# leimao/Voice-Converter-CycleGAN

Hardware: NVIDIA H100
Metric: CycleGAN-VC train steps/sec @ batch 256x[24,128] MCEP (higher is better)
Workload: dtype f16f8 (forward / data gradient: fp16 MMA + two e4m3 cross-term MMAs = 2 MMA units per product; weight gradient: fp16 MMA alone, 1 unit; f32 accumulate)

## Files before the change

voice-converter-cyclegan_b200/csrc/engine.cu:

```cuda
#include "../../include/cgvc.h"
#include "kernels.cuh"
#include "tc_gemm.cuh"
#include "geom.h"

#include <atomic>
#include <dlfcn.h>
#include <limits.h>
#include <stddef.h>
#include <math.h>
#include <stdarg.h>
#include <stdio.h>
#include <string.h>

#include <map>
#include <string>
#include <utility>
#include <vector>

static thread_local std::string g_create_error;

#define ADAM_B1 0.5f
#define ADAM_B2 0.999f
#define ADAM_EPS 1e-8f

// ... 371 lines not shown

static int conv_fwd(cgvc_engine* e, const Layer& L, const LayerTensors& t, const ConvIO& io, float* P, cudaStream_t st) {
  bool done = false;
  if (t.tc && io.xhi)
    RET(tc_result(e, tc_conv_fwd(*t.tc, t.precision, t.debug, io.xhi, io.xlo, io.n, io.H, io.W, L.sh, L.sw, P, st, nullptr, nullptr, packed(io)),
                  &L.a, "forward", &done));
  if (done) return 0;
  if (L.gated() && L.a.cin == 1 && io.x && !io.pk.off && L.a.cout % 4 == 0 && 256 % (L.a.cout / 2) == 0) {
    GatherGeom g = fwd_geom(io.n, io.H, io.W, L.a.kh, L.a.kw, L.sh, L.sw);
    CK(launch_conv_c1_fwd(g, io.x, t.ka, t.kg, t.ba, t.bg, L.a.cout, P, st));
    return 0;
  }
  RET(conv_fwd_simt(e, t.ka, t.ba, L.a, L.sh, L.sw, io, P, L.width(), 0, st));
  if (L.gated()) RET(conv_fwd_simt(e, t.kg, t.bg, L.g, L.sh, L.sw, io, P, L.width(), L.a.cout, st));
  return 0;
}

static int conv_dgrad(cgvc_engine* e, const Layer& L, const LayerTensors& t, const ConvIO& io, const float* dP, PlanePair dp, float* dx,
                      int accumulate, cudaStream_t st, const TcBwdFuse* fuse = nullptr, bool* fused = nullptr) {
  bool done = false;
  if (t.tc && dp.hi)
    RET(tc_result(e, tc_conv_dgrad(*t.tc, t.precision, t.debug, dp.hi, dp.lo, io.n, io.H, io.W, L.sh, L.sw, dx, accumulate, st, fuse, fused,
                                   packed(io)), &L.a, "data gradient", &done));
  if (done) return 0;
  RET(conv_dgrad_simt(e, t.ka, L.a, L.sh, L.sw, io.n, io.H, io.W, dP, L.width(), 0, dx, accumulate, st, packed(io)));
  if (L.gated()) RET(conv_dgrad_simt(e, t.kg, L.g, L.sh, L.sw, io.n, io.H, io.W, dP, L.width(), L.a.cout, dx, 1, st, packed(io)));
  return 0;
}

static int conv_wgrad(cgvc_engine* e, const Layer& L, const LayerTensors& t, const ConvIO& io, const float* dP, PlanePair dp, cudaStream_t st,
                      const DetSlab* det) {
  bool done = false;
  if (t.tc && dp.hi && io.xhi)
    RET(tc_result(e, tc_conv_wgrad(*t.tc, t.precision, t.wgrad16, io.xhi, io.xlo, dp.hi, dp.lo, io.n, io.H, io.W, L.sh, L.sw, t.dka, t.dkg,
                                   st, det, packed(io)), &L.a, "weight gradient", &done));
  if (done) return 0;
  RET(conv_wgrad_simt(e, t.dka, L.a, L.sh, L.sw, io, dP, L.width(), 0, st, det));
  if (L.gated()) RET(conv_wgrad_simt(e, t.dkg, L.g, L.sh, L.sw, io, dP, L.width(), L.a.cout, st, det));
  return 0;
}

static PostParams post_params(const cgvc_engine* e, const Layer& L, const LayerTensors& t, const ConvIO& io, const GLAct& A,
                              int rows_per_sample_out, bool keep_y, float* scratch, const float* resid = nullptr) {
  PostParams q; memset(&q, 0, sizeof q);
  q.scratch = scratch;
  q.p = A.P; q.ldp = L.width(); q.Cc = L.a.cout; q.B = io.n; q.sh = L.shuffle;
  q.R = rows_per_sample_out * L.shuffle; q.C = L.a.cout / L.shuffle;
  q.has_in = L.has_in; q.has_gate = L.gated();
  q.beta_a = t.beta_a; q.gamma_a = t.gamma_a; q.beta_g = t.beta_g; q.gamma_g = t.gamma_g;
  q.resid = resid;
  q.y = (keep_y || !A.Yhi) ? A.Y : nullptr;
  q.stats = L.has_in ? A.stats : nullptr; q.y_hi = A.Yhi; q.y_lo = A.Ylo;
  q.qmode = t.precision == CGVC_PREC_F16F8;
  q.sat = sat_act(e);
  if (io.pk.off && L.has_in && io.seg_out) {
    const long long frames = (long long)io.pk.div * io.W, view_rows = q.R;
    q.B = io.pk.n; q.R = (int)(view_rows * io.pk.max_len / frames);
    q.seg = PackGeom{io.seg_out, io.pk.n, 1, q.R}; q.seg_rows = view_rows;
  } else if (io.pk.off && L.has_in) {
    const long long view_rows = q.R;
    const int div = (int)((long long)io.pk.div * io.W / view_rows);
    q.seg = PackGeom{io.pk.off, io.pk.n, div, io.pk.max_len}; q.seg_rows = view_rows;
    q.B = io.pk.n; q.R = io.pk.max_len / div;
  }
  return q;
}

// ... 236 lines not shown
                    float* dx, int accumulate, cudaStream_t st, const Layer* up, const LayerTensors* ut, const GLAct* upA) {
  const int other = 1 - w.cur;
  TcBwdFuse f;
  const bool fuse = up && w.fuse && dp.hi;
  if (fuse) f = bwd_fuse(*up, *ut, *upA, in.W, w.pb[other]);
  bool fused = false;
  RET(conv_dgrad(e, L, t, in, dP, dp, dx, accumulate, st, fuse ? &f : nullptr, &fused));
  if (fused) w.have = other;
  return 0;
}

static int layer_backward(cgvc_engine* e, BwdWalk& w, const Layer& L, const GLAct& A, const ConvIO& in, const float* dy,
                          int rows_per_sample_out, bool wgrad, float* dx, int accumulate, cudaStream_t st,
                          const Layer* up = nullptr, const GLAct* upA = nullptr) {
  const LayerTensors t = layer_tensors(e, L, wgrad);
  PostBwdParams q;
  RET(layer_dp(e, w, L, t, A, dy, in.n, rows_per_sample_out, st, q, &in));
  const PlanePair dp{q.dp_hi, q.dp_lo};
  if (wgrad) RET(run_wgrad(w.S, dp.hi != nullptr, st, [&](cudaStream_t ws) { return conv_wgrad(e, L, t, in, q.dp, dp, ws, det_of(w.S)); }));
  if (!dx) return 0;
  LayerTensors ut{};
  if (up) ut = layer_tensors(e, *up, wgrad);
  return layer_dx(e, w, L, t, in, q.dp, dp, dx, accumulate, st, up, &ut, upA);
}

static int o1_edge_backward(cgvc_engine* e, const GenNet& N, const float* d_out, const __nv_bfloat16* uhi, const __nv_bfloat16* ulo, int n,
                            int T, PlanePair dz, float* du, const BwdScratch& S, cudaStream_t st, const long long* off = nullptr, int n_off = 0) {
  const int nf = e->cfg.num_features;
  float* Gm = e->G();
  const TcLayer& O = e->tcw.layers[N.o1f_slot];
  CK(launch_im2col_taps(d_out, (long long)n * T, T, nf, N.o1.a.kw, -1, edge_cpad(N.o1.a.kw * nf), e->cfg.precision == CGVC_PREC_F16F8,
                        dz.hi, dz.lo, st, off, n_off, sat_grad(e), ufl_grad(e)));
  RET(run_wgrad(S, true, st, [&](cudaStream_t ws) {
    return tc_result(e, tc_conv_wgrad(O, e->cfg.precision, e->tcw.wgrad16, uhi, ulo, dz.hi, dz.lo, n, 1, T, 1, 1, Gm + N.o1.a.k, nullptr, ws,
                                      det_of(S)),
                     &N.o1.a, "weight gradient (tap-lowered)"); }));
  RET(tc_result(e, tc_conv_dgrad(O, e->cfg.precision, e->tcw.debug, dz.hi, dz.lo, n, 1, T, 1, 1, du, 0, st), &N.o1.a,
                "data gradient (tap-lowered)"));
  return 0;
}

static int h1_edge_backward(cgvc_engine* e, const GenNet& N, const __nv_bfloat16* xchi, const __nv_bfloat16* xclo, PlanePair dp, int n,
                            int T, float* dz, float* dx, const BwdScratch& S, cudaStream_t st, const long long* off = nullptr, int n_off = 0) {
  const int nf = e->cfg.num_features;
  float* Gm = e->G();
  const TcLayer& H = e->tcw.layers[N.h1c_slot];
  RET(run_wgrad(S, true, st, [&](cudaStream_t ws) {
    return tc_result(e, tc_conv_wgrad(H, e->cfg.precision, e->tcw.wgrad16, xchi, xclo, dp.hi, dp.lo, n, 1, T, 1, 1, Gm + N.h1.a.k,
                                      Gm + N.h1.g.k, ws, det_of(S)),
                     &N.h1.a, "weight gradient (tap-lowered)"); }));
  if (dz) RET(tc_result(e, tc_conv_dgrad(H, e->cfg.precision, e->tcw.debug, dp.hi, dp.lo, n, 1, T, 1, 1, dz, 0, st), &N.h1.a,
                        "data gradient (tap-lowered)"));
  if (dz && dx) CK(launch_col2im_taps(dz, N.h1.a.kw * nf, (long long)n * T, T, nf, N.h1.a.kw, -1, nullptr, dx, st, off, n_off));
  return 0;
}

static int generator_backward(cgvc_engine* e, const GenNet& N, const GenActs& A, const float* d_out_cl, float* d_in_cl,
                              const BwdScratch& S, cudaStream_t st) {
  const bool packed = A.off != nullptr;
  const int n = packed ? 1 : A.n, T = packed ? (int)A.rows : A.T, nf = e->cfg.num_features;
  float* Gm = e->G();
  auto at = [&](const float* x, const __nv_bfloat16* hi, const __nv_bfloat16* lo, int W) {
    ConvIO io; io.x = x; io.xhi = hi; io.xlo = lo; io.n = n; io.H = 1; io.W = W;
    if (packed) io.pk = PackGeom{A.off, A.n, (int)(A.rows / W), A.max_len};
    return io;
  };
  auto of = [&](const GLAct& a, int W) { return at(a.Y, a.Yhi, a.Ylo, W); };
  BwdWalk w(S, e->opt.fuse_bwd && !packed && !e->opt.deterministic && !sat_grad(e) && !side_on(S) && tc_enabled(e) && S.dPhi && S.dP2hi &&
               A.r[0].h1.Yhi && A.r[0].h2.Yhi);
  const bool edge = edge_on(e, N) && A.xchi && A.z;
  CK(launch_colsum(d_out_cl, (long long)n * T, nf, 0, nf, Gm + N.o1.a.b, st, det_of(S)));
  const ConvIO u2 = of(A.u[1], T);
  if (edge && u2.xhi && S.dPhi) {
    RET(o1_edge_backward(e, N, d_out_cl, u2.xhi, u2.xlo, n, T, dp_planes(w, st), S.bufA, S, st, A.off, A.n));
  } else {
    const LayerTensors t = layer_tensors(e, N.o1, true);
    PlanePair dp{nullptr, nullptr};
    if (t.tc && u2.xhi && S.dPhi) {
      dp = dp_planes(w, st);
      CK(tc_split_planes(e->cfg.precision, d_out_cl, (long long)n * T, nf, dp.hi, dp.lo, st, sat_grad(e), ufl_grad(e)));
    }
// ... 1788 lines not shown
```

voice-converter-cyclegan_b200/csrc/tc_gemm.cu:

```cuda
#include "tc_gemm.cuh"
#include "geom.h"
#include "kernels.cuh"
#include "wgmma.cuh"

#include <cuda.h>
#include <stdint.h>
#include <stdio.h>
#include <string.h>

namespace {

typedef CUresult (*EncodeTiledFn)(CUtensorMap*, CUtensorMapDataType, cuuint32_t, void*, const cuuint64_t*, const cuuint64_t*,
                                  const cuuint32_t*, const cuuint32_t*, CUtensorMapInterleave, CUtensorMapSwizzle,
                                  CUtensorMapL2promotion, CUtensorMapFloatOOBfill);
EncodeTiledFn get_encoder() {
  static EncodeTiledFn fn = nullptr;
  if (!fn) {
    void* p = nullptr; cudaDriverEntryPointQueryResult q;
    if (cudaGetDriverEntryPoint("cuTensorMapEncodeTiled", &p, cudaEnableDefault, &q) == cudaSuccess && q == cudaDriverEntryPointSuccess)
      fn = (EncodeTiledFn)p;
  }
  return fn;
}
bool make_tmap3(CUtensorMap* m, const void* base, uint64_t d0, uint64_t d1, uint64_t d2, uint32_t b1) {
// ... 141 lines not shown
__device__ __forceinline__ RowPos nt_row(const TcNTParams& p, long long m) {
  RowPos r;
  r.y = (int)fdiv((uint32_t)m, p.div_bw);
  const uint32_t rem = (uint32_t)m - (uint32_t)r.y * p.div_bw.d;
  r.b = (int)fdiv(rem, p.div_w);
  r.x = (int)(rem - (uint32_t)r.b * p.div_w.d);
  return r;
}
template <int PK = 0>
__device__ __forceinline__ uint32_t nt_tile_taps(const TcNTParams& p, long long m0, long long M) {
  const long long m1 = m0 + 127 < M ? m0 + 127 : M - 1;
  if constexpr (PK == 2) {
    const int dout = p.pk.div * p.g.sx;
    const Pack2Pos a = pack2_pos(p.pk, p.g.Hy, dout, m0), b = pack2_pos(p.pk, p.g.Hy, dout, m1);
    return a.u == b.u ? gather_tap_mask(p.g, a.y, b.y) : (1u << p.g.ntaps) - 1u;
  }
  return gather_tap_mask(p.g, nt_row(p, m0).y, nt_row(p, m1).y);
}

struct TcTNParams {
  GatherGeom g;
  const __nv_bfloat16 *x_hi, *x_lo; int x_ld; int C;
  const __nv_bfloat16 *g_hi, *g_lo; int g_ld; int N;
  float* dw_a; float* dw_g; int n_split;
  int ksplit;
  FastDiv div_hw, div_w;
  CUtensorMap tm_g_hi, tm_g_lo;
  const uint8_t *x8_hi, *x8_lo;
  const uint8_t *g8_hi, *g8_lo;
  int w16;
  int fold_n;
  float* part; long long part_k, numel_a;
  PackGeom pk;
};

__device__ __forceinline__ float* tn_dst(float* base, int slab, int C, int c, int ncols, int col, int fold_n) {
  if (fold_n) { const int t = col / fold_n; return base + ((long long)t * C + c) * fold_n + (col - t * fold_n); }
  return base + ((long long)slab * C + c) * ncols + col;
}

constexpr int kProducerThreads = 128;


template <int BN, int NPL>
struct NTCfg {
  static constexpr int A_PLANE = 128 * 128;
  static constexpr int B_PLANE = BN * 128;
  static constexpr int PLANES = NPL == 2 ? 2 : 1;
  static constexpr int STAGE = PLANES * (A_PLANE + B_PLANE);
  static constexpr int STAGES = (192 * 1024) / STAGE;
  static constexpr int SMEM = STAGES * STAGE + 1024;
  static_assert(STAGES * STAGE >= 128 * BN * 4, "the finished fp32 tile is staged over the pipeline stages");
};

template <int BN>
__device__ __forceinline__ int acc_off(int r, int n) { return r * BN + (n & ~31) + ((((n >> 2) & 7) ^ (r & 7)) << 2) + (n & 3); }
template <int BN>
__device__ __forceinline__ void acc_ld32(const float* acc, int r, int col, uint32_t (&v)[32]) {
#pragma unroll
  for (int c = 0; c < 8; ++c) {
    const float4 x = *reinterpret_cast<const float4*>(acc + r * BN + col + ((c ^ (r & 7)) << 2));
    v[4 * c] = __float_as_uint(x.x); v[4 * c + 1] = __float_as_uint(x.y); v[4 * c + 2] = __float_as_uint(x.z); v[4 * c + 3] = __float_as_uint(x.w);
  }
}

__device__ __forceinline__ float warp_colsum32(float (&t)[32], int lane) {
#pragma unroll
// ... 753 lines not shown
      const int r0 = wg * 64 + (tw >> 5) * 16 + ((tw & 31) >> 2), c0 = 2 * (tw & 3);
      if constexpr (EPI == 0) {
        if (!(p.debug & 3)) nt_store_fragments<BN, PK>(p, d, M, m0, n0, r0, c0);
      } else {
        consumer_bar();
        if (!(p.debug & 2)) {
#pragma unroll
          for (int j = 0; j < BN / 8; ++j) {
            *reinterpret_cast<float2*>(acc_s + acc_off<BN>(r0, 8 * j + c0)) = make_float2(d[4 * j], d[4 * j + 1]);
            *reinterpret_cast<float2*>(acc_s + acc_off<BN>(r0 + 8, 8 * j + c0)) = make_float2(d[4 * j + 2], d[4 * j + 3]);
          }
        }
        consumer_bar();
        nt_tile_epilogue<BN, NPL, EPI>(p, M, m0, n0, cw & 3, lane, epi_stage[cw], epi_rowp[cw], epi_bc[cw], epi_xch[wg], acc_s, wg, 2);
        fence_proxy_async();
        __syncwarp();
        if (lane == 0) mbar_arrive(&acc_free_bar);
      }
    }
  }
}

#define CGVC_Q_WGRAD_SHIFT 12
template <int NPL, int W16>
struct TNCfg {
  static constexpr int A_PLANE = 64 * 256;
  static constexpr int B_PLANE = 64 * 512;
  static constexpr int PLANES = (NPL == 1 || W16) ? 1 : 2;
  static constexpr int STAGE = PLANES * (A_PLANE + B_PLANE);
  static constexpr int STAGES = (192 * 1024) / STAGE;
  static constexpr int SMEM = STAGES * STAGE + 1024;
};

template <int NPL, int W16, int DET, int PK = 0>
__global__ void __launch_bounds__(kNTThreads, 1)
tc_gg_tn_kernel(const __grid_constant__ TcTNParams p) {
  static_assert(W16 == 0 || NPL == 3, "the fp16-only weight gradient is a form of CGVC_PREC_F16F8");
  using Cfg = TNCfg<NPL, W16>;
  constexpr int S = Cfg::STAGES;
  constexpr int BN = 256;
  extern __shared__ uint8_t smem_raw[];
  __shared__ __align__(8) uint64_t full_bar[S], empty_bar[S];

  const uint32_t smem_base = (smem_u32(smem_raw) + 1023u) & ~1023u;
  const int warp = threadIdx.x >> 5, lane = threadIdx.x & 31;
  const GatherGeom& g = p.g;
  const long long M = (long long)g.B * g.Hy * g.Wx;
  const int HW = g.Hy * g.Wx;
  const int n_tiles = (p.g_ld + BN - 1) / BN, c_tiles = (p.x_ld + 127) / 128;
  const int num_items = n_tiles * c_tiles * g.ntaps * p.ksplit;
  constexpr int pass0 = (NPL == 3 && !W16) ? 0 : 1;
  long long chunk_rows = (M + p.ksplit - 1) / p.ksplit;
  chunk_rows = (chunk_rows + 63) / 64 * 64;

  struct Item { int n0, c0, tap, ks; long long mbeg, mend; int num_kb; };
  auto decode = [&](int item) -> Item {
    Item w;
    int n_t = item % n_tiles; int t1 = item / n_tiles;
    int c_t = t1 % c_tiles; int t2 = t1 / c_tiles;
    w.tap = t2 % g.ntaps; const int ks = t2 / g.ntaps; w.ks = ks;
    w.n0 = n_t * BN; w.c0 = c_t * 128;
    w.mbeg = (long long)ks * chunk_rows;
    w.mend = (w.mbeg + chunk_rows < M) ? w.mbeg + chunk_rows : M;
    w.num_kb = w.mend > w.mbeg ? (int)((w.mend - w.mbeg + 63) / 64) : 0;
    return w;
  };

  if (threadIdx.x == 0) {
    for (int s = 0; s < S; ++s) { mbar_init(&full_bar[s], kProducerThreads + 1); mbar_init(&empty_bar[s], 8); }
    fence_barrier_init();
    tma_prefetch_desc(&p.tm_g_hi);
    if (NPL == 2) tma_prefetch_desc(&p.tm_g_lo);
  }
  __syncthreads();

  if (warp < 4) {
    const int t = threadIdx.x;
    const int chunk = t & 7, rsub = t >> 3;
    int stage = 0; uint32_t phase = 0;
    for (int item = blockIdx.x; item < num_items; item += gridDim.x) {
      const Item w = decode(item);
      for (int pass = pass0; pass < 2; ++pass)
      for (int kb = 0; kb < w.num_kb; ++kb) {
        mbar_wait(&empty_bar[stage], phase ^ 1);
        const uint32_t sA = smem_base + stage * Cfg::STAGE;
        const uint32_t sB = sA + Cfg::PLANES * Cfg::A_PLANE;
        long long xoff[4];
#pragma unroll
        for (int i = 0; i < 4; ++i) {
          const long long m = w.mbeg + (long long)kb * 64 + rsub + 16 * i;
          xoff[i] = -1;
          if (m < w.mend) {
            if constexpr (PK == 2) {
              const Pack2Pos o = pack2_pos(p.pk, g.Hy, p.pk.div * g.sx, m);
              const long long r = pack2_row(o.o0, o.o1, g.Hs, p.pk.div, o.y * g.sy + g.oy[w.tap], o.x * g.sx + g.ox[w.tap]);
              if (r >= 0) xoff[i] = r * p.x_ld + w.c0 + chunk * 8;
            } else if constexpr (PK) {
              const int dout = p.pk.div * g.sx;
              const int u = pack_find(p.pk.off, p.pk.n, m * dout);
              const long long o0 = __ldg(p.pk.off + u), o1 = __ldg(p.pk.off + u + 1);
              const int xx = (int)(m - o0 / dout) * g.sx + g.ox[w.tap];
              if (xx >= 0 && xx < (int)((o1 - o0) / p.pk.div)) xoff[i] = (o0 / p.pk.div + xx) * p.x_ld + w.c0 + chunk * 8;
            } else {
              const uint32_t mu = (uint32_t)m;
              int b = (int)fdiv(mu, p.div_hw); int rem = (int)(mu - (uint32_t)b * (uint32_t)HW);
              int y = (int)fdiv((uint32_t)rem, p.div_w); int x = rem - y * g.Wx;
              int yy = y * g.sy + g.oy[w.tap], xx = x * g.sx + g.ox[w.tap];
              if (yy >= 0 && yy < g.Hs && xx >= 0 && xx < g.Ws)
                xoff[i] = ((long long)(b * g.Hs + yy) * g.Ws + xx) * p.x_ld + w.c0 + chunk * 8;
            }
          }
        }
        if (NPL == 3 && pass == 0) {
#pragma unroll
          for (int i = 0; i < 4; ++i) {
            const int kr = rsub + 16 * i;
            const uint32_t so = sw128(kr, chunk);
#pragma unroll
            for (int a = 0; a < 2; ++a) {
              const bool ok = xoff[i] >= 0 && (w.c0 + a * 64) < p.x_ld;
              uint2 vh = make_uint2(0u, 0u), vl = make_uint2(0u, 0u);
              if (ok) { vh = __ldg(reinterpret_cast<const uint2*>(p.x8_hi + xoff[i] + a * 64)); vl = __ldg(reinterpret_cast<const uint2*>(p.x8_lo + xoff[i] + a * 64)); }
              st_shared16(sA + a * 8192 + so, e4m3x8_to_f16x8(vh));
              st_shared16(sA + Cfg::A_PLANE + a * 8192 + so, e4m3x8_to_f16x8(vl));
            }
            const long long m = w.mbeg + (long long)kb * 64 + kr;
#pragma unroll
            for (int a = 0; a < 4; ++a) {
              const int col = w.n0 + a * 64 + chunk * 8;
              const bool ok = m < w.mend && col < p.g_ld;
              uint2 vh = make_uint2(0u, 0u), vl = make_uint2(0u, 0u);
              if (ok) { vh = __ldg(reinterpret_cast<const uint2*>(p.g8_hi + m * p.g_ld + col)); vl = __ldg(reinterpret_cast<const uint2*>(p.g8_lo + m * p.g_ld + col)); }
              st_shared16(sB + a * 8192 + so, e4m3x8_to_f16x8(vh));
              st_shared16(sB + Cfg::B_PLANE + a * 8192 + so, e4m3x8_to_f16x8(vl));
            }
          }
          fence_proxy_async();
          if (t == 0) mbar_expect_tx(&full_bar[stage], 0);
          mbar_arrive(&full_bar[stage]);
        } else {
          if (t == 0) {
            const int row0 = (int)(w.mbeg + (long long)kb * 64);
            int natoms = 0;
#pragma unroll
            for (int a = 0; a < 4; ++a) natoms += (w.n0 + a * 64) < p.g_ld ? 1 : 0;
            mbar_expect_tx(&full_bar[stage], (NPL == 2 ? 2 : 1) * natoms * 8192);
#pragma unroll
            for (int a = 0; a < 4; ++a) {
              if ((w.n0 + a * 64) < p.g_ld) {
                tma_load3(sB + a * 8192, &p.tm_g_hi, w.n0 + a * 64, row0, 0, &full_bar[stage]);
                if (NPL == 2) tma_load3(sB + Cfg::B_PLANE + a * 8192, &p.tm_g_lo, w.n0 + a * 64, row0, 0, &full_bar[stage]);
              }
            }
          }
#pragma unroll
          for (int i = 0; i < 4; ++i) {
            const uint32_t so = sw128(rsub + 16 * i, chunk);
#pragma unroll
            for (int a = 0; a < 2; ++a) {
              const bool ok = xoff[i] >= 0 && (w.c0 + a * 64) < p.x_ld;
              const long long off = ok ? xoff[i] + a * 64 : 0;
              cp_async16(sA + a * 8192 + so, p.x_hi + off, ok ? 16u : 0u);
              if (NPL == 2) cp_async16(sA + Cfg::A_PLANE + a * 8192 + so, p.x_lo + off, ok ? 16u : 0u);
            }
          }
          cp_async_arrive_noinc(&full_bar[stage]);
        }
        if (++stage == S) { stage = 0; phase ^= 1; }
      }
    }
  } else {
    const int cw = warp - 4;
    const int wg = cw >> 2;
    const int tw = threadIdx.x - 128 * (wg + 1);
    int stage = 0; uint32_t phase = 0;
    for (int item = blockIdx.x; item < num_items; item += gridDim.x) {
      const Item w = decode(item);
      if (w.num_kb == 0) continue;
      float d[BN / 2];
#pragma unroll
      for (int i = 0; i < BN / 2; ++i) d[i] = 0.f;
      int prev = -1;
      if constexpr (NPL == 3 && !W16) {
        consume_stages<BN, MMA_F16_CROSS, 1, Cfg>(d, w.num_kb, stage, phase, prev, full_bar, empty_bar, smem_base, wg, lane);
        rescale_acc(d, 1.f / (float)(1 << CGVC_Q_WGRAD_SHIFT));
        consume_stages<BN, MMA_F16, 1, Cfg>(d, w.num_kb, stage, phase, prev, full_bar, empty_bar, smem_base, wg, lane);
      } else if constexpr (NPL == 3) {
// ... 251 lines not shown
  }
  else if (p.pk.off) {
    if (epi != 0 || p.g.B != 1 || p.g.Hy != 1) return cudaErrorInvalidValue;
    const int npl = precision == 3 ? 3 : x3 ? 2 : 1;
    if (bn == 256)      { if (npl == 3) LAUNCH_NT(256, 3, 0, 1); else if (npl == 2) LAUNCH_NT(256, 2, 0, 1); else LAUNCH_NT(256, 1, 0, 1); }
    else if (bn == 128) { if (npl == 3) LAUNCH_NT(128, 3, 0, 1); else if (npl == 2) LAUNCH_NT(128, 2, 0, 1); else LAUNCH_NT(128, 1, 0, 1); }
    else                { if (npl == 3) LAUNCH_NT(32, 3, 0, 1);  else if (npl == 2) LAUNCH_NT(32, 2, 0, 1);  else LAUNCH_NT(32, 1, 0, 1); }
  }
  else {
    const bool ta = nt_tma_maps(p, precision == 3 ? 3 : x3 ? 2 : 1);
#define LAUNCH_NT_D(BN_, NPL_, EPI_) do { if (ta) LAUNCH_NT(BN_, NPL_, EPI_, 0, 1); else LAUNCH_NT(BN_, NPL_, EPI_); } while (0)
    if (precision == 3) {
      if (epi == 1)       LAUNCH_NT_D(256, 3, 1);
      else if (epi == 2)  LAUNCH_NT_D(256, 3, 2);
      else if (epi == 5)  LAUNCH_NT_D(256, 3, 5);
      else if (epi != 0)  return cudaErrorInvalidValue;
      else if (bn == 256) LAUNCH_NT_D(256, 3, 0);
      else if (bn == 128) LAUNCH_NT_D(128, 3, 0);
      else                LAUNCH_NT_D(32, 3, 0);
    }
    else if (epi == 1)  { if (x3) LAUNCH_NT_D(256, 2, 1); else LAUNCH_NT_D(256, 1, 1); }
    else if (epi == 2)  { if (x3) LAUNCH_NT_D(256, 2, 2); else LAUNCH_NT_D(256, 1, 2); }
    else if (epi == 3)  { if (x3) LAUNCH_NT_D(256, 2, 3); else LAUNCH_NT_D(256, 1, 3); }
    else if (epi == 4)  { if (x3) LAUNCH_NT_D(256, 2, 4); else LAUNCH_NT_D(256, 1, 4); }
    else if (epi == 5)  { if (x3) LAUNCH_NT_D(256, 2, 5); else LAUNCH_NT_D(256, 1, 5); }
    else if (bn == 256) { if (x3) LAUNCH_NT_D(256, 2, 0); else LAUNCH_NT_D(256, 1, 0); }
    else if (bn == 128) { if (x3) LAUNCH_NT_D(128, 2, 0); else LAUNCH_NT_D(128, 1, 0); }
    else                { if (x3) LAUNCH_NT_D(32, 2, 0);  else LAUNCH_NT_D(32, 1, 0); }
#undef LAUNCH_NT_D
  }
#undef LAUNCH_NT
  prof_end(st);
  return cudaGetLastError();
}

cudaError_t launch_tn(TcTNParams p, int precision, cudaStream_t st, const DetSlab* det) {
  const long long M = (long long)p.g.B * p.g.Hy * p.g.Wx;
  if (M == 0) return cudaSuccess;
  if (M >= (1ll << 31)) return cudaErrorInvalidValue;
  const int tiles = ((p.g_ld + 255) / 256) * ((p.x_ld + 127) / 128) * p.g.ntaps;
  const int nsm = num_sms();
  long long maxsplit = M / 1024; if (maxsplit < 1) maxsplit = 1; if (maxsplit > 32) maxsplit = 32;
  int ksplit = 1; double best = 0.0;
  for (int ks = 1; ks <= (int)maxsplit; ++ks) {
    long long items = (long long)tiles * ks;
    double eff = (double)items / (double)(((items + nsm - 1) / nsm) * nsm);
    if (items < nsm) eff *= 0.5;
    if (eff > best + 0.02) { best = eff; ksplit = ks; }
  }
  const long long numel = (long long)p.g.ntaps * p.C * p.N;
  auto chunk_of = [&](int ks) { return ((M + ks - 1) / ks + 63) / 64 * 64; };
  if (det && det->p)
    while (ksplit > 1 && ((long long)ksplit * numel > det->cap || (long long)(ksplit - 1) * chunk_of(ksplit) >= M)) --ksplit;
  const bool det_split = det && det->p && ksplit > 1;
  if (det_split) { p.part = det->p; p.part_k = numel; p.numel_a = (long long)p.g.ntaps * p.C * p.n_split; }
  p.ksplit = ksplit;
  p.div_hw = make_fastdiv((uint32_t)(p.g.Hy * p.g.Wx)); p.div_w = make_fastdiv((uint32_t)p.g.Wx);
  const long long items = (long long)tiles * ksplit;
  dim3 grid((unsigned)(items < nsm ? items : nsm));
  cudaError_t e;
  ++g_cgvc_launches;
  prof_begin(st, 2.0 * (double)M * p.N * p.g.ntaps * p.C, 1, M, p.N, p.g.ntaps * p.C);
#define LAUNCH_TN(NPL_, W16_, DET_, ...)                                                                      \
  do {                                                                                                        \
    e = set_smem(tc_gg_tn_kernel<NPL_, W16_, DET_, ##__VA_ARGS__>, TNCfg<NPL_, W16_>::SMEM);                  \
    if (e != cudaSuccess) return e;                                                                           \
    tc_gg_tn_kernel<NPL_, W16_, DET_, ##__VA_ARGS__><<<grid, kNTThreads, TNCfg<NPL_, W16_>::SMEM, st>>>(p);   \
  } while (0)
  if (p.pk.off && (p.g.Hy > 1 || p.g.Hs > 1)) {
    if (p.g.B != 1) return cudaErrorInvalidValue;
    if (det_split) {
      if (precision == 3) { if (p.w16) LAUNCH_TN(3, 1, 1, 2); else LAUNCH_TN(3, 0, 1, 2); }
      else if (precision == 1) LAUNCH_TN(2, 0, 1, 2);
      else                     LAUNCH_TN(1, 0, 1, 2);
    } else {
      if (precision == 3) { if (p.w16) LAUNCH_TN(3, 1, 0, 2); else LAUNCH_TN(3, 0, 0, 2); }
      else if (precision == 1) LAUNCH_TN(2, 0, 0, 2);
      else                     LAUNCH_TN(1, 0, 0, 2);
    }
  } else if (p.pk.off) {
    if (p.g.B != 1 || p.g.Hy != 1) return cudaErrorInvalidValue;
    if (det_split) {
      if (precision == 3) { if (p.w16) LAUNCH_TN(3, 1, 1, 1); else LAUNCH_TN(3, 0, 1, 1); }
      else if (precision == 1) LAUNCH_TN(2, 0, 1, 1);
      else                     LAUNCH_TN(1, 0, 1, 1);
    } else {
      if (precision == 3) { if (p.w16) LAUNCH_TN(3, 1, 0, 1); else LAUNCH_TN(3, 0, 0, 1); }
      else if (precision == 1) LAUNCH_TN(2, 0, 0, 1);
      else                     LAUNCH_TN(1, 0, 0, 1);
    }
  } else if (det_split) {
    if (precision == 3) { if (p.w16) LAUNCH_TN(3, 1, 1); else LAUNCH_TN(3, 0, 1); }
    else if (precision == 1) LAUNCH_TN(2, 0, 1);
    else                     LAUNCH_TN(1, 0, 1);
  } else {
    if (precision == 3) { if (p.w16) LAUNCH_TN(3, 1, 0); else LAUNCH_TN(3, 0, 0); }
    else if (precision == 1) LAUNCH_TN(2, 0, 0);
    else                     LAUNCH_TN(1, 0, 0);
  }
#undef LAUNCH_TN
  prof_end(st);
  if (!det_split) return cudaGetLastError();
  e = cudaGetLastError();
  if (e != cudaSuccess) return e;
  return launch_reduce_parts(p.part, ksplit, numel, DetSegs{{p.dw_a, p.dw_g}, {0, p.numel_a}, {p.numel_a, p.dw_g ? numel - p.numel_a : 0}}, st);
}

inline int ru(int v, int m) { return (v + m - 1) / m * m; }
inline int Ntot(const TcLayer& L) { return L.cout * (L.gated ? 2 : 1); }
inline int cin_k(const TcLayer& L) { return ru(L.cin, 64); }
inline int cin_n(const TcLayer& L) { return ru(L.cin, 128); }
inline int nt_k(const TcLayer& L) { return ru(Ntot(L), 64); }
inline int nt_n(const TcLayer& L) { return ru(Ntot(L), 128); }
inline int cin_q(const TcLayer& L) { return ru(L.cin, 128); }
inline int nt_q(const TcLayer& L) { return ru(Ntot(L), 128); }
inline size_t wq_elems(const TcLayer& L) { return (size_t)L.kh * L.kw * nt_n(L) * cin_q(L); }
inline size_t wdq_elems(const TcLayer& L) { return (size_t)L.kh * L.kw * cin_n(L) * nt_q(L); }
inline size_t wf_elems(const TcLayer& L) { return (size_t)L.kh * L.kw * nt_n(L) * cin_k(L); }
inline size_t wd_elems(const TcLayer& L) { return (size_t)L.kh * L.kw * cin_n(L) * nt_k(L); }
inline int layer_perm(const TcLayer& L) {
  if (L.gated && L.shuffle == 2 && L.cout % 128 == 0) return 2;
  return (L.gated && L.cout % 128 == 0) ? 1 : 0;
}
inline bool layer_ok(const TcLayer& L) {
  if (L.fold && (L.gated || L.kh * L.kw != 1 || L.cout % L.fold || (L.cout / L.fold) % 4)) return false;
  return L.kh * L.kw <= CGVC_MAX_TAPS && Ntot(L) % 4 == 0;
}
inline bool layer_ok_q(const TcLayer& L) { return layer_ok(L) && L.cin % 4 == 0; }


bool make_layer_maps(TcLayer& L) {
// ... 93 lines not shown
  int epi = 0;
  if (fuse && fuse->R > 0 && gs.size() == 1 && H == 1 && sh == 1 && sw == 1 && (fuse->R == 32 || fuse->R == 64 || fuse->R == 128) &&
      gs[0].Wx == fuse->R && cin_n(L) % 256 == 0 && L.cin == cin_n(L) && fuse->bp && fuse->stats && fuse->dp_hi && fuse->dp_lo && fuse->gamma_a &&
      (fuse->gated ? (fuse->gamma_g && fuse->beta_a && fuse->beta_g) : (dx != nullptr)) && precision != 3)
    epi = fuse->gated ? 3 : 4;
  for (const GatherGeom& g : gs) {
    TcNTParams p; memset(&p, 0, sizeof p);
    p.g = g;
    if (pk) {
      p.pk = *pk; p.pk.div = pk->div * sw;
    }
    p.a_hi = dPhi; p.a_lo = dPlo; p.a_ld = nt_k(L); p.C = nt_k(L);
    p.b_hi = L.wd_hi; p.b_lo = L.wd_lo; p.Nw = cin_n(L); p.N = L.cin;
    p.dst = dx; p.d_ld = L.cin; p.bias = nullptr; p.accumulate = accumulate;
    p.tm_b_hi = L.tm_d_hi; p.tm_b_lo = L.tm_d_lo; p.debug = debug;
    if (precision == 3) {
      p.a_ld = nt_q(L); p.C = nt_q(L); p.a_lo = nullptr;
      p.a8_hi = reinterpret_cast<const uint8_t*>(dPlo); p.a8_lo = p.a8_hi + (size_t)g.B * g.Hs * g.Ws * nt_q(L);
      p.tm_b_hi = L.tm_dq16; p.tm_b8_hi = L.tm_dq8hi; p.tm_b8_lo = L.tm_dq8lo;
    }
    if (epi) {
      p.R = fuse->R; p.C_out = L.cin; p.stats = const_cast<float*>(fuse->stats);
      p.gamma_a = fuse->gamma_a; p.beta_a = fuse->beta_a; p.gamma_g = fuse->gamma_g; p.beta_g = fuse->beta_g;
      p.bp = fuse->bp; p.bp_ld = fuse->bp_ld; p.dp_hi = fuse->dp_hi; p.dp_lo = fuse->dp_lo; p.dp_ld = fuse->dp_ld;
      p.dbeta_a = fuse->dbeta_a; p.dgamma_a = fuse->dgamma_a; p.dbeta_g = fuse->dbeta_g; p.dgamma_g = fuse->dgamma_g;
    }
    cudaError_t e = launch_nt(p, precision, st, epi);
    if (e != cudaSuccess) return (int)e;
  }
  if (fused_out) *fused_out = epi != 0;
  return 0;
}

int tc_conv_wgrad(const TcLayer& L, int precision, int w16, const __nv_bfloat16* xhi, const __nv_bfloat16* xlo,
                  const __nv_bfloat16* dPhi, const __nv_bfloat16* dPlo, int n, int H, int W, int sh, int sw,
                  float* dwa, float* dwg, cudaStream_t st, const DetSlab* det, const PackGeom* pk) {
  if (!layer_ok(L) || (precision == 3 && !layer_ok_q(L))) return TC_UNSUPPORTED;
  if (pk && (n != 1 || (H == 1 && L.kh != 1))) return (int)cudaErrorInvalidValue;
  TcTNParams p; memset(&p, 0, sizeof p);
  if (pk) p.pk = *pk;
  p.w16 = (precision == 3 && w16) ? 1 : 0;
  p.fold_n = L.fold ? L.cout / L.fold : 0;
  p.g = fwd_geom(n, H, W, L.kh, L.kw, sh, sw);
  p.x_hi = xhi; p.x_lo = xlo; p.x_ld = cin_k(L); p.C = L.cin;
  p.g_hi = dPhi; p.g_lo = dPlo; p.g_ld = nt_k(L); p.N = Ntot(L);
  p.dw_a = dwa; p.dw_g = dwg; p.n_split = L.cout;
  const long long M = (long long)p.g.B * p.g.Hy * p.g.Wx;
  if (precision == 3) {
    const long long rows_in = (long long)n * H * W;
    p.x_ld = cin_q(L); p.g_ld = nt_q(L); p.x_lo = p.g_lo = nullptr;
    p.x8_hi = reinterpret_cast<const uint8_t*>(xlo); p.x8_lo = p.x8_hi + rows_in * p.x_ld;
    p.g8_hi = reinterpret_cast<const uint8_t*>(dPlo); p.g8_lo = p.g8_hi + M * p.g_ld;
    if (!make_tmap3_t(&p.tm_g_hi, dPhi, CU_TENSOR_MAP_DATA_TYPE_FLOAT16, 2, (uint64_t)p.g_ld, (uint64_t)M, 1, 64, 64))
      return (int)cudaErrorInvalidValue;
  } else if (!make_tmap3(&p.tm_g_hi, dPhi, (uint64_t)nt_k(L), (uint64_t)M, 1, 64) || !make_tmap3(&p.tm_g_lo, dPlo, (uint64_t)nt_k(L), (uint64_t)M, 1, 64)) {
    return (int)cudaErrorInvalidValue;
  }
  return (int)launch_tn(p, precision, st, det);
}

int tc_register(TcWeights& w, size_t ka, size_t kg, size_t ba, size_t bg, int kh, int kw, int cin, int cout, int gated, int shuffle, int fold) {
  TcLayer L{}; L.ka = ka; L.kg = kg; L.ba = ba; L.bg = bg; L.kh = kh; L.kw = kw; L.cin = cin; L.cout = cout; L.gated = gated; L.shuffle = shuffle; L.fold = fold;
  w.layers.push_back(L);
  return (int)w.layers.size() - 1;
}

static cudaError_t tc_init_kernels();

int tc_alloc(TcWeights& w, int precision, bool train) {
  { cudaError_t ie = tc_init_kernels(); if (ie != cudaSuccess) return (int)ie; }
  w.quant = precision == 3;
  w.quant_bwd = w.quant && train;
  w.wgrad16 = w.quant;
  size_t total = 0;
// ... 51 lines not shown
      err = cudaMalloc(&w.prep_jobs, jobs.size() * sizeof(PrepJob));
      if (err != cudaSuccess) return (int)err;
      err = cudaMemcpy(w.prep_jobs, jobs.data(), jobs.size() * sizeof(PrepJob), cudaMemcpyHostToDevice);
      if (err != cudaSuccess) return (int)err;
    }
  }
  w.ready = false;
  return 0;
}

static cudaError_t tc_init_kernels() {
  cudaError_t e;
#define INIT_NT(BN_, NPL_, EPI_) if ((e = set_smem(tc_gg_nt_kernel<BN_, NPL_, EPI_>, NTCfg<BN_, NPL_>::SMEM)) != cudaSuccess) return e;
  INIT_NT(256, 2, 0) INIT_NT(256, 1, 0) INIT_NT(128, 2, 0) INIT_NT(128, 1, 0) INIT_NT(32, 2, 0) INIT_NT(32, 1, 0)
  INIT_NT(256, 2, 1) INIT_NT(256, 1, 1) INIT_NT(256, 2, 2) INIT_NT(256, 1, 2)
  INIT_NT(256, 2, 3) INIT_NT(256, 1, 3) INIT_NT(256, 2, 4) INIT_NT(256, 1, 4) INIT_NT(256, 2, 5) INIT_NT(256, 1, 5)
  INIT_NT(256, 3, 0) INIT_NT(128, 3, 0) INIT_NT(32, 3, 0) INIT_NT(256, 3, 1) INIT_NT(256, 3, 2) INIT_NT(256, 3, 5)
#undef INIT_NT
#define INIT_NT(BN_, NPL_, EPI_) if ((e = set_smem(tc_gg_nt_kernel<BN_, NPL_, EPI_, 0, 1>, NTCfg<BN_, NPL_>::SMEM)) != cudaSuccess) return e;
  INIT_NT(256, 2, 0) INIT_NT(256, 1, 0) INIT_NT(128, 2, 0) INIT_NT(128, 1, 0) INIT_NT(32, 2, 0) INIT_NT(32, 1, 0)
  INIT_NT(256, 2, 1) INIT_NT(256, 1, 1) INIT_NT(256, 2, 2) INIT_NT(256, 1, 2)
  INIT_NT(256, 2, 3) INIT_NT(256, 1, 3) INIT_NT(256, 2, 4) INIT_NT(256, 1, 4) INIT_NT(256, 2, 5) INIT_NT(256, 1, 5)
  INIT_NT(256, 3, 0) INIT_NT(128, 3, 0) INIT_NT(32, 3, 0) INIT_NT(256, 3, 1) INIT_NT(256, 3, 2) INIT_NT(256, 3, 5)
#undef INIT_NT
#define INIT_NT_PK(BN_, NPL_, PK_) if ((e = set_smem(tc_gg_nt_kernel<BN_, NPL_, 0, PK_>, NTCfg<BN_, NPL_>::SMEM)) != cudaSuccess) return e;
  INIT_NT_PK(256, 1, 1) INIT_NT_PK(256, 2, 1) INIT_NT_PK(256, 3, 1) INIT_NT_PK(128, 1, 1) INIT_NT_PK(128, 2, 1) INIT_NT_PK(128, 3, 1)
  INIT_NT_PK(32, 1, 1) INIT_NT_PK(32, 2, 1) INIT_NT_PK(32, 3, 1)
  INIT_NT_PK(256, 1, 2) INIT_NT_PK(256, 2, 2) INIT_NT_PK(256, 3, 2) INIT_NT_PK(128, 1, 2) INIT_NT_PK(128, 2, 2) INIT_NT_PK(128, 3, 2)
  INIT_NT_PK(32, 1, 2) INIT_NT_PK(32, 2, 2) INIT_NT_PK(32, 3, 2)
#undef INIT_NT_PK
#define INIT_TN(NPL_, W16_, DET_) if ((e = set_smem(tc_gg_tn_kernel<NPL_, W16_, DET_>, TNCfg<NPL_, W16_>::SMEM)) != cudaSuccess) return e;
  INIT_TN(3, 1, 0) INIT_TN(3, 0, 0) INIT_TN(2, 0, 0) INIT_TN(1, 0, 0)
  INIT_TN(3, 1, 1) INIT_TN(3, 0, 1) INIT_TN(2, 0, 1) INIT_TN(1, 0, 1)
#define INIT_TN_PK(NPL_, W16_, DET_, PK_) if ((e = set_smem(tc_gg_tn_kernel<NPL_, W16_, DET_, PK_>, TNCfg<NPL_, W16_>::SMEM)) != cudaSuccess) return e;
  INIT_TN_PK(3, 1, 0, 1) INIT_TN_PK(3, 0, 0, 1) INIT_TN_PK(2, 0, 0, 1) INIT_TN_PK(1, 0, 0, 1)
  INIT_TN_PK(3, 1, 1, 1) INIT_TN_PK(3, 0, 1, 1) INIT_TN_PK(2, 0, 1, 1) INIT_TN_PK(1, 0, 1, 1)
  INIT_TN_PK(3, 1, 0, 2) INIT_TN_PK(3, 0, 0, 2) INIT_TN_PK(2, 0, 0, 2) INIT_TN_PK(1, 0, 0, 2)
  INIT_TN_PK(3, 1, 1, 2) INIT_TN_PK(3, 0, 1, 2) INIT_TN_PK(2, 0, 1, 2) INIT_TN_PK(1, 0, 1, 2)
#undef INIT_TN_PK
#undef INIT_TN
  return cudaSuccess;
}

void tc_free(TcWeights& w) {
  if (w.pool) cudaFree(w.pool);
  if (w.prep_jobs) cudaFree(w.prep_jobs);
  w.pool = nullptr; w.prep_jobs = nullptr; w.ready = false;
}

static int refresh_jobs(TcWeights& w, const float* params, int j0, int j1, cudaStream_t st) {
  if (j1 <= j0) return 0;
  const int b0 = w.job_first[j0], nb = w.job_first[j1] - b0;
  ++g_cgvc_launches;
  prep_weights_q_all_kernel<<<(unsigned)nb, 256, 0, st>>>(params, (const PrepJob*)w.prep_jobs, j0, j1, b0);
  return (int)cudaGetLastError();
}

int tc_refresh_weights(TcWeights& w, const float* params, cudaStream_t st) {
  if (!w.pool) return 0;
  const bool batched = w.prep_batched && w.prep_jobs;
  for (TcLayer& L : w.layers) {
    if (batched && L.wq16) continue;
    int r = tc_refresh_layer(L, params + L.ka, params + L.kg, params + L.ba, params + L.bg, st);
    if (r != 0) return r;
  }
  if (batched) { int r = refresh_jobs(w, params, 0, (int)w.job_ka.size(), st); if (r != 0) return r; }
// ... 87 lines not shown
```

voice-converter-cyclegan_b200/csrc/tc_gemm.cuh:

```cuda
#pragma once
#include <cuda.h>
#include <cuda_runtime.h>
#include <cuda_bf16.h>
#include <stddef.h>
#include <vector>
#include "kernels.cuh"

#define TC_UNSUPPORTED (-12345)

struct TcLayer {
  size_t ka, kg, ba, bg;
  int kh, kw, cin, cout, gated;
  int shuffle;
  int fold;
  __nv_bfloat16 *wf_hi, *wf_lo;
  __nv_bfloat16 *wd_hi, *wd_lo;
  float* bias;
  CUtensorMap tm_f_hi, tm_f_lo;
  CUtensorMap tm_d_hi, tm_d_lo;
  void* wq16; uint8_t *wq8hi, *wq8lo;
  CUtensorMap tm_q16, tm_q8hi, tm_q8lo;
  void* wdq16; uint8_t *wdq8hi, *wdq8lo;
  CUtensorMap tm_dq16, tm_dq8hi, tm_dq8lo;
};
// ... 18 lines not shown
  const float *gamma_a, *beta_a, *gamma_g, *beta_g;
  float* stats;
  const float* resid;
  float* y; __nv_bfloat16 *y_hi, *y_lo;
};

struct TcBwdFuse {
  int R;
  int gated;
  const float* bp; int bp_ld;
  const float* stats;
  const float *gamma_a, *beta_a, *gamma_g, *beta_g;
  __nv_bfloat16 *dp_hi, *dp_lo; int dp_ld;
  float *dbeta_a, *dgamma_a, *dbeta_g, *dgamma_g;
};

int tc_register(TcWeights& w, size_t ka, size_t kg, size_t ba, size_t bg, int kh, int kw, int cin, int cout, int gated, int shuffle = 1, int fold = 0);
int tc_alloc(TcWeights& w, int precision, bool train);
void tc_free(TcWeights& w);
int tc_refresh_weights(TcWeights& w, const float* params, cudaStream_t st);
int tc_refresh_layer(TcLayer& L, const float* ka, const float* kg, const float* ba, const float* bg, cudaStream_t st);
int tc_refresh_weights_range(TcWeights& w, const float* params, size_t begin, size_t end, cudaStream_t st);
void tc_layer_dims(const TcWeights& w, int slot, int dims[7]);
int tc_layer_plane(const TcWeights& w, int slot, const char* name, const void** p, size_t* bytes);

cudaError_t tc_split_planes(int precision, const float* x, long long rows, int C, __nv_bfloat16* hi, __nv_bfloat16* lo, cudaStream_t st,
                            unsigned long long* sat = nullptr, unsigned long long* ufl = nullptr);

int tc_conv_fwd(const TcLayer& L, int precision, int debug, const __nv_bfloat16* xhi, const __nv_bfloat16* xlo, int n, int H, int W,
                int sh, int sw, float* P, cudaStream_t st, const TcFuse* fuse = nullptr, bool* fused = nullptr, const PackGeom* pk = nullptr);
int tc_conv_dgrad(const TcLayer& L, int precision, int debug, const __nv_bfloat16* dPhi, const __nv_bfloat16* dPlo, int n, int H, int W,
                  int sh, int sw, float* dx, int accumulate, cudaStream_t st, const TcBwdFuse* fuse = nullptr, bool* fused = nullptr,
                  const PackGeom* pk = nullptr);
int tc_conv_wgrad(const TcLayer& L, int precision, int w16, const __nv_bfloat16* xhi, const __nv_bfloat16* xlo,
                  const __nv_bfloat16* dPhi, const __nv_bfloat16* dPlo, int n, int H, int W, int sh, int sw,
                  float* dwa, float* dwg, cudaStream_t st, const DetSlab* det = nullptr,
                  const PackGeom* pk = nullptr);

void tc_profile_enable(int on);
bool tc_profile_is_on();
int tc_profile_collect(double ms[3], double flops[3], long long launches[3]);
int tc_profile_launches(double* ms, double* flops, long long* meta4, int capacity, int* n_out);
```

Measured before the change: 10.74.

## Load weight-gradient activation tiles with TMA instead of producer-thread gathers

Adds a TMA variant of the weight-gradient TN kernel in which one producer warp issues 4D tensor-map loads for the activation planes and 3D loads for the gradient planes, replacing the four-warp manual gather and swizzled shared-memory stores. It is used for dense (unpacked) layers when the geometry fits the box constraints and the precision does not need e4m3 widening, including the fp16-only weight-gradient mode. This is meant to cut producer instruction and register overhead and let the async copy engine keep the pipeline fed. It also threads a debug flag through so activation loads can be skipped for timing experiments, and it adds more kernel instantiations plus tensor-map setup on the host for each launch.

```diff
diff --git a/voice-converter-cyclegan_b200/csrc/engine.cu b/voice-converter-cyclegan_b200/csrc/engine.cu
--- a/voice-converter-cyclegan_b200/csrc/engine.cu
+++ b/voice-converter-cyclegan_b200/csrc/engine.cu
@@ -427,7 +427,7 @@
                       const DetSlab* det) {
   bool done = false;
   if (t.tc && dp.hi && io.xhi)
-    RET(tc_result(e, tc_conv_wgrad(*t.tc, t.precision, t.wgrad16, io.xhi, io.xlo, dp.hi, dp.lo, io.n, io.H, io.W, L.sh, L.sw, t.dka, t.dkg,
+    RET(tc_result(e, tc_conv_wgrad(*t.tc, t.precision, t.debug, t.wgrad16, io.xhi, io.xlo, dp.hi, dp.lo, io.n, io.H, io.W, L.sh, L.sw, t.dka, t.dkg,
                                    st, det, packed(io)), &L.a, "weight gradient", &done));
   if (done) return 0;
   RET(conv_wgrad_simt(e, t.dka, L.a, L.sh, L.sw, io, dP, L.width(), 0, st, det));
@@ -730,7 +730,7 @@
   CK(launch_im2col_taps(d_out, (long long)n * T, T, nf, N.o1.a.kw, -1, edge_cpad(N.o1.a.kw * nf), e->cfg.precision == CGVC_PREC_F16F8,
                         dz.hi, dz.lo, st, off, n_off, sat_grad(e), ufl_grad(e)));
   RET(run_wgrad(S, true, st, [&](cudaStream_t ws) {
-    return tc_result(e, tc_conv_wgrad(O, e->cfg.precision, e->tcw.wgrad16, uhi, ulo, dz.hi, dz.lo, n, 1, T, 1, 1, Gm + N.o1.a.k, nullptr, ws,
+    return tc_result(e, tc_conv_wgrad(O, e->cfg.precision, e->tcw.debug, e->tcw.wgrad16, uhi, ulo, dz.hi, dz.lo, n, 1, T, 1, 1, Gm + N.o1.a.k, nullptr, ws,
                                       det_of(S)),
                      &N.o1.a, "weight gradient (tap-lowered)"); }));
   RET(tc_result(e, tc_conv_dgrad(O, e->cfg.precision, e->tcw.debug, dz.hi, dz.lo, n, 1, T, 1, 1, du, 0, st), &N.o1.a,
@@ -744,7 +744,7 @@
   float* Gm = e->G();
   const TcLayer& H = e->tcw.layers[N.h1c_slot];
   RET(run_wgrad(S, true, st, [&](cudaStream_t ws) {
-    return tc_result(e, tc_conv_wgrad(H, e->cfg.precision, e->tcw.wgrad16, xchi, xclo, dp.hi, dp.lo, n, 1, T, 1, 1, Gm + N.h1.a.k,
+    return tc_result(e, tc_conv_wgrad(H, e->cfg.precision, e->tcw.debug, e->tcw.wgrad16, xchi, xclo, dp.hi, dp.lo, n, 1, T, 1, 1, Gm + N.h1.a.k,
                                       Gm + N.h1.g.k, ws, det_of(S)),
                      &N.h1.a, "weight gradient (tap-lowered)"); }));
   if (dz) RET(tc_result(e, tc_conv_dgrad(H, e->cfg.precision, e->tcw.debug, dp.hi, dp.lo, n, 1, T, 1, 1, dz, 0, st), &N.h1.a,
diff --git a/voice-converter-cyclegan_b200/csrc/tc_gemm.cu b/voice-converter-cyclegan_b200/csrc/tc_gemm.cu
--- a/voice-converter-cyclegan_b200/csrc/tc_gemm.cu
+++ b/voice-converter-cyclegan_b200/csrc/tc_gemm.cu
@@ -197,7 +197,10 @@
   int fold_n;
   float* part; long long part_k, numel_a;
   PackGeom pk;
+  int debug;
+  CUtensorMap tm_x_hi, tm_x_lo;
 };
+static_assert(sizeof(TcTNParams) <= 4096, "kernel parameters are limited to 4 KB");
 
 __device__ __forceinline__ float* tn_dst(float* base, int slab, int C, int c, int ncols, int col, int fold_n) {
   if (fold_n) { const int t = col / fold_n; return base + ((long long)t * C + c) * fold_n + (col - t * fold_n); }
@@ -1017,10 +1020,11 @@
   static constexpr int SMEM = STAGES * STAGE + 1024;
 };
 
-template <int NPL, int W16, int DET, int PK = 0>
+template <int NPL, int W16, int DET, int PK = 0, int TA = 0>
 __global__ void __launch_bounds__(kNTThreads, 1)
 tc_gg_tn_kernel(const __grid_constant__ TcTNParams p) {
   static_assert(W16 == 0 || NPL == 3, "the fp16-only weight gradient is a form of CGVC_PREC_F16F8");
+  static_assert(!TA || (!PK && (NPL != 3 || W16)), "the TMA form is dense and loads the planes as they are (no e4m3 widening)");
   using Cfg = TNCfg<NPL, W16>;
   constexpr int S = Cfg::STAGES;
   constexpr int BN = 256;
@@ -1052,14 +1056,54 @@
   };
 
   if (threadIdx.x == 0) {
-    for (int s = 0; s < S; ++s) { mbar_init(&full_bar[s], kProducerThreads + 1); mbar_init(&empty_bar[s], 8); }
+    for (int s = 0; s < S; ++s) { mbar_init(&full_bar[s], TA ? 1 : kProducerThreads + 1); mbar_init(&empty_bar[s], 8); }
     fence_barrier_init();
     tma_prefetch_desc(&p.tm_g_hi);
     if (NPL == 2) tma_prefetch_desc(&p.tm_g_lo);
+    if (TA) { tma_prefetch_desc(&p.tm_x_hi); if (NPL == 2) tma_prefetch_desc(&p.tm_x_lo); }
   }
   __syncthreads();
 
-  if (warp < 4) {
+  if (TA && warp < 4) {
+    if (warp == 0) {
+      const int box_rows = (g.Hy == 1 || g.Wx >= 64) ? 64 : g.Wx;
+      const int nbox = 64 / box_rows;
+      const uint32_t x_bytes = (p.debug & 4) ? 0u : (uint32_t)Cfg::PLANES * Cfg::A_PLANE;
+      int stage = 0; uint32_t phase = 0;
+      for (int item = blockIdx.x; item < num_items; item += gridDim.x) {
+        const Item w = decode(item);
+        for (int kb = 0; kb < w.num_kb; ++kb) {
+          mbar_wait(&empty_bar[stage], phase ^ 1);
+          const uint32_t sA = smem_base + stage * Cfg::STAGE;
+          const uint32_t sB = sA + Cfg::PLANES * Cfg::A_PLANE;
+          const int row0 = (int)(w.mbeg + (long long)kb * 64);
+          if (lane == 0) {
+            int natoms = 0;
+#pragma unroll
+            for (int a = 0; a < 4; ++a) natoms += (w.n0 + a * 64) < p.g_ld ? 1 : 0;
+            mbar_expect_tx(&full_bar[stage], Cfg::PLANES * natoms * 8192 + x_bytes);
+          }
+          __syncwarp();
+          if (lane < 4) {
+            if ((w.n0 + lane * 64) < p.g_ld) {
+              tma_load3(sB + lane * 8192, &p.tm_g_hi, w.n0 + lane * 64, row0, 0, &full_bar[stage]);
+              if (NPL == 2) tma_load3(sB + Cfg::B_PLANE + lane * 8192, &p.tm_g_lo, w.n0 + lane * 64, row0, 0, &full_bar[stage]);
+            }
+          } else if (x_bytes && lane < 4 + 2 * nbox) {
+            const int j = (lane - 4) >> 1, a = (lane - 4) & 1;
+            const uint32_t mu = (uint32_t)(row0 + j * box_rows);
+            const int b = (int)fdiv(mu, p.div_hw); const int rem = (int)(mu - (uint32_t)b * (uint32_t)HW);
+            const int y = (int)fdiv((uint32_t)rem, p.div_w); const int x = rem - y * g.Wx;
+            const int c0 = w.c0 + a * 64, xs = x * g.sx + g.ox[w.tap], ys = y * g.sy + g.oy[w.tap];
+            const uint32_t dst = sA + a * 8192 + j * box_rows * 128;
+            tma_load4(dst, &p.tm_x_hi, c0, xs, ys, b, &full_bar[stage]);
+            if (NPL == 2) tma_load4(dst + Cfg::A_PLANE, &p.tm_x_lo, c0, xs, ys, b, &full_bar[stage]);
+          }
+          if (++stage == S) { stage = 0; phase ^= 1; }
+        }
+      }
+    }
+  } else if (warp < 4) {
     const int t = threadIdx.x;
     const int chunk = t & 7, rsub = t >> 3;
     int stage = 0; uint32_t phase = 0;
@@ -1103,6 +1147,7 @@
             const uint32_t so = sw128(kr, chunk);
 #pragma unroll
             for (int a = 0; a < 2; ++a) {
+              if (p.debug & 4) break;
               const bool ok = xoff[i] >= 0 && (w.c0 + a * 64) < p.x_ld;
               uint2 vh = make_uint2(0u, 0u), vl = make_uint2(0u, 0u);
               if (ok) { vh = __ldg(reinterpret_cast<const uint2*>(p.x8_hi + xoff[i] + a * 64)); vl = __ldg(reinterpret_cast<const uint2*>(p.x8_lo + xoff[i] + a * 64)); }
@@ -1138,6 +1183,7 @@
               }
             }
           }
+          if (!(p.debug & 4))
 #pragma unroll
           for (int i = 0; i < 4; ++i) {
             const uint32_t so = sw128(rsub + 16 * i, chunk);
@@ -1455,6 +1501,14 @@
 #undef LAUNCH_NT
   prof_end(st);
   return cudaGetLastError();
+}
+
+static bool tn_tma_maps(TcTNParams& p, int npl) {
+  const GatherGeom& g = p.g;
+  const int wx = g.Wx < 64 ? g.Wx : 64;
+  if (g.Wx < 8 || 64 % wx || g.Wx % wx || wx * g.sx > 256 || g.sx > 8) return false;
+  const uint32_t bx = (uint32_t)(wx * g.sx), nb = g.Hy == 1 ? (uint32_t)(64 / wx) : 1u;
+  return make_tmap_act(&p.tm_x_hi, p.x_hi, 2, p.x_ld, g, bx, nb) && (npl != 2 || make_tmap_act(&p.tm_x_lo, p.x_lo, 2, p.x_ld, g, bx, nb));
 }
 
 cudaError_t launch_tn(TcTNParams p, int precision, cudaStream_t st, const DetSlab* det) {
@@ -1512,14 +1566,19 @@
       else if (precision == 1) LAUNCH_TN(2, 0, 0, 1);
       else                     LAUNCH_TN(1, 0, 0, 1);
     }
-  } else if (det_split) {
-    if (precision == 3) { if (p.w16) LAUNCH_TN(3, 1, 1); else LAUNCH_TN(3, 0, 1); }
-    else if (precision == 1) LAUNCH_TN(2, 0, 1);
-    else                     LAUNCH_TN(1, 0, 1);
   } else {
-    if (precision == 3) { if (p.w16) LAUNCH_TN(3, 1, 0); else LAUNCH_TN(3, 0, 0); }
-    else if (precision == 1) LAUNCH_TN(2, 0, 0);
-    else                     LAUNCH_TN(1, 0, 0);
+    const bool ta = (precision != 3 || p.w16) && tn_tma_maps(p, precision == 1 ? 2 : 1);
+#define LAUNCH_TN_D(NPL_, W16_, DET_) do { if (ta) LAUNCH_TN(NPL_, W16_, DET_, 0, 1); else LAUNCH_TN(NPL_, W16_, DET_); } while (0)
+    if (det_split) {
+      if (precision == 3) { if (p.w16) LAUNCH_TN_D(3, 1, 1); else LAUNCH_TN(3, 0, 1); }
+      else if (precision == 1) LAUNCH_TN_D(2, 0, 1);
+      else                     LAUNCH_TN_D(1, 0, 1);
+    } else {
+      if (precision == 3) { if (p.w16) LAUNCH_TN_D(3, 1, 0); else LAUNCH_TN(3, 0, 0); }
+      else if (precision == 1) LAUNCH_TN_D(2, 0, 0);
+      else                     LAUNCH_TN_D(1, 0, 0);
+    }
+#undef LAUNCH_TN_D
   }
 #undef LAUNCH_TN
   prof_end(st);
@@ -1679,14 +1738,14 @@
   return 0;
 }
 
-int tc_conv_wgrad(const TcLayer& L, int precision, int w16, const __nv_bfloat16* xhi, const __nv_bfloat16* xlo,
+int tc_conv_wgrad(const TcLayer& L, int precision, int debug, int w16, const __nv_bfloat16* xhi, const __nv_bfloat16* xlo,
                   const __nv_bfloat16* dPhi, const __nv_bfloat16* dPlo, int n, int H, int W, int sh, int sw,
                   float* dwa, float* dwg, cudaStream_t st, const DetSlab* det, const PackGeom* pk) {
   if (!layer_ok(L) || (precision == 3 && !layer_ok_q(L))) return TC_UNSUPPORTED;
   if (pk && (n != 1 || (H == 1 && L.kh != 1))) return (int)cudaErrorInvalidValue;
   TcTNParams p; memset(&p, 0, sizeof p);
   if (pk) p.pk = *pk;
-  p.w16 = (precision == 3 && w16) ? 1 : 0;
+  p.w16 = (precision == 3 && w16) ? 1 : 0; p.debug = debug;
   p.fold_n = L.fold ? L.cout / L.fold : 0;
   p.g = fwd_geom(n, H, W, L.kh, L.kw, sh, sw);
   p.x_hi = xhi; p.x_lo = xlo; p.x_ld = cin_k(L); p.C = L.cin;
@@ -1804,6 +1863,10 @@
 #define INIT_TN(NPL_, W16_, DET_) if ((e = set_smem(tc_gg_tn_kernel<NPL_, W16_, DET_>, TNCfg<NPL_, W16_>::SMEM)) != cudaSuccess) return e;
   INIT_TN(3, 1, 0) INIT_TN(3, 0, 0) INIT_TN(2, 0, 0) INIT_TN(1, 0, 0)
   INIT_TN(3, 1, 1) INIT_TN(3, 0, 1) INIT_TN(2, 0, 1) INIT_TN(1, 0, 1)
+#define INIT_TN_TA(NPL_, W16_, DET_) if ((e = set_smem(tc_gg_tn_kernel<NPL_, W16_, DET_, 0, 1>, TNCfg<NPL_, W16_>::SMEM)) != cudaSuccess) return e;
+  INIT_TN_TA(3, 1, 0) INIT_TN_TA(2, 0, 0) INIT_TN_TA(1, 0, 0)
+  INIT_TN_TA(3, 1, 1) INIT_TN_TA(2, 0, 1) INIT_TN_TA(1, 0, 1)
+#undef INIT_TN_TA
 #define INIT_TN_PK(NPL_, W16_, DET_, PK_) if ((e = set_smem(tc_gg_tn_kernel<NPL_, W16_, DET_, PK_>, TNCfg<NPL_, W16_>::SMEM)) != cudaSuccess) return e;
   INIT_TN_PK(3, 1, 0, 1) INIT_TN_PK(3, 0, 0, 1) INIT_TN_PK(2, 0, 0, 1) INIT_TN_PK(1, 0, 0, 1)
   INIT_TN_PK(3, 1, 1, 1) INIT_TN_PK(3, 0, 1, 1) INIT_TN_PK(2, 0, 1, 1) INIT_TN_PK(1, 0, 1, 1)
diff --git a/voice-converter-cyclegan_b200/csrc/tc_gemm.cuh b/voice-converter-cyclegan_b200/csrc/tc_gemm.cuh
--- a/voice-converter-cyclegan_b200/csrc/tc_gemm.cuh
+++ b/voice-converter-cyclegan_b200/csrc/tc_gemm.cuh
@@ -74,7 +74,7 @@
 int tc_conv_dgrad(const TcLayer& L, int precision, int debug, const __nv_bfloat16* dPhi, const __nv_bfloat16* dPlo, int n, int H, int W,
                   int sh, int sw, float* dx, int accumulate, cudaStream_t st, const TcBwdFuse* fuse = nullptr, bool* fused = nullptr,
                   const PackGeom* pk = nullptr);
-int tc_conv_wgrad(const TcLayer& L, int precision, int w16, const __nv_bfloat16* xhi, const __nv_bfloat16* xlo,
+int tc_conv_wgrad(const TcLayer& L, int precision, int debug, int w16, const __nv_bfloat16* xhi, const __nv_bfloat16* xlo,
                   const __nv_bfloat16* dPhi, const __nv_bfloat16* dPlo, int n, int H, int W, int sh, int sw,
                   float* dwa, float* dwg, cudaStream_t st, const DetSlab* det = nullptr,
                   const PackGeom* pk = nullptr);
```

After: 11.24, median of 6. 4.7% higher.
